# weitianxin/MACR

Measured on AMD Instinct MI355X. Metric: train interactions/sec + eval users/sec (full-catalog top-K@20), higher is better.
Workload: dtype f32; 1 GPU; gowalla-shape MACR-MF rubibceboth d=64 batch=4096 c=40 (n_users=29858, n_items=40981); synthetic Xavier tables, Zipf positives, batches as sampled (grouped on the device inside the step); parallelism=replicas x1 (train) / item-sharded x1 + RCCL all-gather (eval), global_batch=4096

## Files before the change

### macr_amd/csrc/eval_kernels.hip

```cpp
#include "common.hpp"

#include <algorithm>

#include <type_traits>

namespace macr {

#ifdef MACR_ABL_COUNT
__device__ unsigned long long g_dbg[8];
#define MACR_DBG_ADD(k, v) do { if ((threadIdx.x & 63) == 0) atomicAdd(&g_dbg[k], (unsigned long long)(v)); } while (0)
#else
#define MACR_DBG_ADD(k, v) do { } while (0)
#endif

typedef float f32x16 __attribute__((ext_vector_type(16)));

constexpr int kCap = 64;
constexpr int kTileItems = 32;
constexpr int kUnitK = 64;
constexpr int kUnitStride = kUnitK + 1;
constexpr int kWavesPerBlock = 8;
constexpr int kUsersPerBlock = 32 * kWavesPerBlock;
constexpr int kSelRegs = 16;

// ... 1055 lines not shown
        if (has_next) store_tile(buf ^ 1);
        __syncthreads();
#pragma unroll
        for (int g = 0; g < UG; ++g) tm_cur[g] = tm_next[g];
        buf ^= 1;
        t = tn; ++vi;
        if (stop) break;
    }
    for (int k = tid; k < kUsersPerBlock; k += THREADS) {
        const int qq = ub * kUsersPerBlock + k;
        const int ql2 = (REPAIR && rl.compact) ? ubv * kUsersPerBlock + k : qq;
        if (qq < U) counts[(size_t)split * rl.stride + ql2] = (int32_t)min(s_cnt[k], (uint32_t)cap);
    }
    }
}

template <int D>
struct StreamCfgC {
    static constexpr int RU = 2 * D / 8 + 1;
    static constexpr int TU = kTileItems * RU;
    static constexpr int NS = D / 16;
    static constexpr int LDU = (TU + 511) / 512, REM = TU - 512 * (LDU - 1);
    static constexpr size_t smem = (size_t)2 * TU * 16 + kUsersPerBlock * 4 + 16;
};
static inline size_t items_c_bytes(int n_local, int d) { return (size_t)n_tiles(n_local) * kTileItems * (2 * d / 8 + 1) * 16; }
template <int D>
struct StreamCfgH1 {
    static constexpr int RU = D / 8 + 1;
    static constexpr int TU = kTileItems * RU;
    static constexpr int NS = D / 16;
    static constexpr int LDU = (TU + 511) / 512, REM = TU - 512 * (LDU - 1);
    static constexpr size_t smem = (size_t)2 * TU * 16 + kUsersPerBlock * 4 + 16;
};
#ifndef MACR_H_TPS
#define MACR_H_TPS 1
#endif
constexpr int kHTiles = MACR_H_TPS;
template <int D>
struct StreamCfgH {
    static constexpr int RU = D / 8 + 1;
    static constexpr int TU = kTileItems * RU;
    static constexpr int NS = D / 16;
    static constexpr int THREADS = 256 * kHTiles;
    static constexpr int SU = kHTiles * TU;
    static constexpr int LDU = (SU + THREADS - 1) / THREADS;
    static constexpr size_t smem = (size_t)2 * SU * 16 + kUsersPerBlock * 4 + 16;
};
__device__ __forceinline__ f32x16 mfma_f16(bf16x8 a, bf16x8 b, f32x16 acc) {
    return __builtin_amdgcn_mfma_f32_32x32x16_f16(__builtin_bit_cast(f16x8, a), __builtin_bit_cast(f16x8, b), acc, 0, 0, 0);
}

template <int KIND> __device__ __forceinline__ bf16x8 bias_query_unit_h(float su, bool on) {
    const float sv = KIND == MACR_SCORE_DIRECT_MINUS_BOTH ? su : 1.0f;
    const uint32_t s1 = f16_rne_bits(sv);
    const float r1 = sv - f16_bits_value(s1);
    const uint32_t s2 = f16_rne_bits(r1), s3 = f16_rne_bits(r1 - f16_bits_value(s2));
    union { uint32_t u[4]; bf16x8 v; } w;
    w.u[0] = on ? (s1 | (s2 << 16)) : 0u; w.u[1] = on ? (s1 | (s3 << 16)) : 0u; w.u[2] = on ? (s2 | (s1 << 16)) : 0u; w.u[3] = 0u;
    return w.v;
}
__device__ __forceinline__ uint4 bias_item_unit_h(float bias) {
    const float bc = fminf(fmaxf(bias, -kHalfMax), kHalfMax);
    const uint32_t b1 = f16_rne_bits(bc);
    const float r1 = bc - f16_bits_value(b1);
    const uint32_t b2 = f16_rne_bits(r1), b3 = f16_rne_bits(r1 - f16_bits_value(b2));
    return make_uint4(b1 | (b1 << 16), b2 | (b1 << 16), b2 | (b3 << 16), 0u);
}
template <int KIND> __device__ __forceinline__ float query_factor_h(float su) { return KIND == MACR_SCORE_RUBI_BOTH ? su : 1.0f; }

template <int KIND> __device__ __forceinline__ float item_scale_c(float sgi) {
    return (KIND == MACR_SCORE_RUBI_BOTH || KIND == MACR_SCORE_RUBI) ? sgi : 1.0f;
}
template <int KIND> __device__ __forceinline__ float item_bias_c(float sgi, float c) {
    return KIND == MACR_SCORE_NORMAL ? 0.0f : -(c * sgi);
}
__device__ __forceinline__ bool sig_u_tiny(float su) { return !(su > 1e-30f); }

template <int D, int KIND, int TRIPS, bool HALF = false, bool FUSED = false>
// ... 523 lines not shown
            one_visit(std::integral_constant<int, 0>(), t, tm_cur);
            store_tile(std::integral_constant<int, 1>());
            __syncthreads();
            tm_cur = tm_next; t = tn; ++vi;
        }
        if (vi >= i1) break;
        {
            const int tn = vi + 1 < i1 ? visit_after(t) : t;
            load_tile(tn);
            __builtin_amdgcn_sched_barrier(0);
            one_visit(std::integral_constant<int, 1>(), t, tm_cur);
            store_tile(std::integral_constant<int, 0>());
            __syncthreads();
            tm_cur = tm_next; t = tn; ++vi;
        }
    }
    if (q_ok && !merge_pairs) {
        float *o = maxima + ((size_t)split * U + q) * 32;
#pragma unroll
        for (int g = 0; g < 4; ++g)
            *reinterpret_cast<float4 *>(o + 8 * g + 4 * h) = make_float4(cmax[4 * g] * fu, cmax[4 * g + 1] * fu, cmax[4 * g + 2] * fu, cmax[4 * g + 3] * fu);
    }
    if (q_ok && merge_pairs) {
        float *o = maxima + ((size_t)split * U + q) * 16 + 8 * h;
        *reinterpret_cast<float4 *>(o) = make_float4(fmaxf(cmax[0], cmax[8]) * fu, fmaxf(cmax[1], cmax[9]) * fu, fmaxf(cmax[2], cmax[10]) * fu,
                                                     fmaxf(cmax[3], cmax[11]) * fu);
        *reinterpret_cast<float4 *>(o + 4) = make_float4(fmaxf(cmax[4], cmax[12]) * fu, fmaxf(cmax[5], cmax[13]) * fu, fmaxf(cmax[6], cmax[14]) * fu,
                                                         fmaxf(cmax[7], cmax[15]) * fu);
    }
    }
}

template <int D, int KIND, bool REPAIR = false>
__global__ __launch_bounds__(StreamCfgH<D>::THREADS, D <= 64 ? 4 : 2) void k_score_stream_h(
    int U, int n_local, const uint4 *__restrict__ users_h, const uint4 *__restrict__ items_h,
    const float *__restrict__ unorm, const uint32_t *__restrict__ qmax_bits,
    const float *__restrict__ sig_u, float c_val, const float *__restrict__ c_dev,
    const uint32_t *__restrict__ mask_bits, const uint32_t *__restrict__ zero_word, int item_offset, int ublocks,
    const float *__restrict__ tau, uint64_t *__restrict__ lists, int32_t *__restrict__ counts, int cap, int32_t *overflow,
    int ovf_per_user, int32_t *blk_flag, const int32_t *__restrict__ ub_map, const int32_t *__restrict__ n_ub_dev, int slots_full) {
    using C = StreamCfgH<D>;
    constexpr int THREADS = C::THREADS, NS = C::NS, RU = C::RU, TU = C::TU, SU = C::SU, LDU = C::LDU;
    constexpr int kCheckTiles = 8;
    const float c = c_dev ? *c_dev : c_val;
    extern __shared__ __align__(16) unsigned char smem[];
    uint4 *s_t = reinterpret_cast<uint4 *>(smem);
    uint32_t *s_cnt = reinterpret_cast<uint32_t *>(smem + (size_t)2 * SU * 16);
    int *s_stop = reinterpret_cast<int *>(s_cnt + kUsersPerBlock);
    const int tid = threadIdx.x, lane = tid & 63, wid = tid >> 6;
    const int col = lane & 31, h = lane >> 5;
    const int tslot = kHTiles == 2 ? __builtin_amdgcn_readfirstlane(wid >> 2) : 0, uw = wid & 3;
    const int T = (n_local + kTileItems - 1) / kTileItems;
    int n_ub = ublocks;
    long long G = gridDim.x;
    const long long b = blockIdx.x;
    RepairLayout rl = {false, 0, U};
    if (REPAIR) {
        n_ub = *n_ub_dev;
        if (n_ub == 0) return;
        rl = repair_layout(slots_full, U, n_ub);
        G = repair_grid(rl, G, ublocks, n_ub, T);
        if (b >= G) return;
    }
    int S = (int)(0.6180339f * (float)T);
    S = S < 1 ? 1 : S;
    for (;; ++S) {
        int x = S, y = T;
        while (y) { const int r = x % y; x = y; y = r; }
        if (x == 1) break;
    }
    auto visit = [&](int i) { return (int)(((unsigned long long)i * (unsigned)S) % (unsigned)T); };
    auto visit_after = [&](int tile) { const int n = tile + S; return n >= T ? n - T : n; };
    const float qmax = __uint_as_float(*qmax_bits);
    const long long W = (long long)n_ub * T;
    const long long w_end = W * (b + 1) / G;
    const size_t mask_stride = mask_bits ? (size_t)U : 0;
    for (long long w = W * b / G; w < w_end;) {
    const int ubv = (int)(w / T), i0 = (int)(w - (long long)ubv * T);
    const int i1 = (int)min((long long)T, i0 + (w_end - w));
    w += i1 - i0;
    long long first = (long long)ubv * T * G / W;
    while (W * (first + 1) / G <= (long long)ubv * T) ++first;
    while (W * first / G > (long long)ubv * T) --first;
    const int split = (int)(b - first);
    const int ub = REPAIR ? ub_map[ubv] : ubv;
    __syncthreads();
    for (int k = tid; k < kUsersPerBlock; k += THREADS) s_cnt[k] = 0u;
    if (tid == 0) *s_stop = 0;
    bf16x8 bq[2][NS], bext[2];
    float thr[2], fu[2];
    uint32_t my_list[2], my_q[2];
    uint32_t *my_cnt[2];
#pragma unroll
    for (int g = 0; g < 2; ++g) {
        const int uslot = uw * 64 + g * 32 + col, q = ub * kUsersPerBlock + uslot;
        const bool q_ok = q < U;
        const uint4 *urow = users_h + (size_t)(q_ok ? q : 0) * (D / 8);
#pragma unroll
        for (int sI = 0; sI < NS; ++sI) {
            uint4 v = urow[2 * sI + h];
            if (!q_ok) v = make_uint4(0u, 0u, 0u, 0u);
            bq[g][sI] = *reinterpret_cast<bf16x8 *>(&v);
        }
        const float su = (score_uses_sig_u(KIND) && q_ok) ? sig_u[q] : 1.0f;
        const bool tiny = KIND == MACR_SCORE_RUBI_BOTH && sig_u_tiny(su);
        fu[g] = query_factor_h<KIND>(su);
        bext[g] = bias_query_unit_h<KIND>(su, KIND != MACR_SCORE_NORMAL && h == 0);
        float tau_s = __builtin_nanf("");
        if (q_ok) tau_s = tau[q] - 1.01f * filter_margin_h(D, unorm[q], qmax, c) * fu[g];
        thr[g] = tau_s / fu[g];
        if (tiny) thr[g] = q_ok ? -INFINITY : thr[g];
        my_list[g] = (uint32_t)((size_t)split * rl.stride + ((REPAIR && rl.compact) ? ubv * kUsersPerBlock + uslot : (q_ok ? q : 0)));
        my_q[g] = mask_bits ? (uint32_t)(q_ok ? q : 0) : 0u;
        my_cnt[g] = &s_cnt[uslot];
    }
    const int id_lane = item_offset + 4 * h;

    uint4 stg[LDU];
    uint32_t tm_next[2] = {0u, 0u};
    auto load_step = [&](int ta, int tb) {
        const int tau_ = __builtin_amdgcn_readfirstlane(ta), tbu = __builtin_amdgcn_readfirstlane(tb);
#pragma unroll
        for (int k = 0; k < LDU; ++k) {
            int e = tid + THREADS * k;
            if (k + 1 == LDU && e >= SU) e -= SU;
            const bool second = kHTiles == 2 && e >= TU;
            stg[k] = items_h[(size_t)(second ? tbu : tau_) * TU + (second ? e - TU : e)];
        }
        const int mine = tslot ? tbu : tau_;
#ifndef MACR_ABL_H_NOMASK
        const uint32_t *mrow = (mask_bits ? mask_bits : zero_word) + (size_t)mine * mask_stride;
        tm_next[0] = mrow[my_q[0]];
        tm_next[1] = mrow[my_q[1]];
#else
        tm_next[0] = zero_word[mine & 0]; tm_next[1] = tm_next[0];
#endif
    };
    auto store_step = [&](auto BUF) {
        constexpr int buf = decltype(BUF)::value;
#pragma unroll
        for (int k = 0; k < LDU; ++k) {
            asm volatile("" : "+v"(stg[k].x), "+v"(stg[k].y), "+v"(stg[k].z), "+v"(stg[k].w));
            if (k + 1 < LDU || tid < SU - THREADS * (LDU - 1)) s_t[buf * SU + tid + THREADS * k] = stg[k];
        }
    };
    auto one_step = [&](auto BUF, int t, uint32_t tm0, uint32_t tm1) {
        constexpr int buf = decltype(BUF)::value;
        const __bf16 *ua = reinterpret_cast<const __bf16 *>(s_t + buf * SU + tslot * TU) + (size_t)col * (8 * RU) + 8 * h;
        f32x16 acc0, acc1;
#pragma unroll
        for (int r = 0; r < 16; ++r) { acc0[r] = 0.f; acc1[r] = 0.f; }
        constexpr int CH = NS < 2 ? NS : (D <= 64 ? 2 : 4);
        bf16x8 ae;
        if (KIND != MACR_SCORE_NORMAL) ae = *reinterpret_cast<const bf16x8 *>(ua - 8 * h + D);
#pragma unroll
        for (int s0 = 0; s0 < NS; s0 += CH) {
            bf16x8 af[CH];
#pragma unroll
            for (int j = 0; j < CH; ++j) af[j] = *reinterpret_cast<const bf16x8 *>(ua + 16 * (s0 + j));
            asm volatile("s_waitcnt lgkmcnt(0)" ::: "memory");
            __builtin_amdgcn_sched_barrier(0);
#pragma unroll
            for (int j = 0; j < CH; ++j) {
#ifndef MACR_ABL_H_NOMFMA
                acc0 = mfma_f16(af[j], bq[0][s0 + j], acc0);
                acc1 = mfma_f16(af[j], bq[1][s0 + j], acc1);
#else
                acc0[j] += (float)af[j][0] * (float)bq[0][s0 + j][0];
                acc1[j] += (float)af[j][1] * (float)bq[1][s0 + j][1];
#endif
            }
            if (KIND != MACR_SCORE_NORMAL && s0 + CH >= NS) {
                acc0 = mfma_f16(ae, bext[0], acc0);
                acc1 = mfma_f16(ae, bext[1], acc1);
            }
            __builtin_amdgcn_sched_barrier(0);
        }
        const int valid = t < 0 ? 0 : n_local - t * kTileItems;
        const uint32_t tailm = valid < kTileItems ? ~0u << (valid > 0 ? valid : 0) : 0u;
        const int id0 = t * kTileItems + id_lane;
        auto epilogue = [&](const f32x16 &acc, uint32_t tm_cur, float thr_g, float fu_g, uint32_t *cnt_g, uint32_t list_g) {
            const uint32_t tmh = (tm_cur | tailm) >> (4 * h);
#pragma unroll
            for (int r4 = 0; r4 < 16; r4 += 4) {
                const float quad = fmaxf(fmaxf(fmaxf(acc[r4], acc[r4 + 1]), acc[r4 + 2]), acc[r4 + 3]);
                if (!__builtin_amdgcn_ballot_w64(quad >= thr_g)) continue;
#pragma unroll
                for (int r = r4; r < r4 + 4; ++r) {
                    const bool above = acc[r] >= thr_g;
                    if (__builtin_amdgcn_ballot_w64(above)) {
                        const int rbit = (r & 3) + 8 * (r >> 2);
                        uint32_t m = tmh;
                        asm volatile("" : "+v"(m));
                        if (above && !((m >> rbit) & 1u)) {
                            const uint32_t pos = atomicAdd(cnt_g, 1u);
                            if (pos < (uint32_t)cap) lists[(size_t)list_g * cap + pos] = make_key(acc[r] * fu_g, id0 + rbit);
                        }
                    }
                }
            }
        };
#ifndef MACR_ABL_H_NOEPI
        epilogue(acc0, tm0, thr[0], fu[0], my_cnt[0], my_list[0]);
        epilogue(acc1, tm1, thr[1], fu[1], my_cnt[1], my_list[1]);
#else
        {
            float m0 = acc0[0], m1 = acc1[0];
#pragma unroll
            for (int r = 1; r < 16; ++r) { m0 = fmaxf(m0, acc0[r]); m1 = fmaxf(m1, acc1[r]); }
            if (m0 == 1.2345e30f || m1 == 1.2345e30f) epilogue(acc0, tm0, thr[0], fu[0], my_cnt[0], my_list[0]);
        }
#endif
    };
    int polled = 0;
    auto stale_mark = [&](int done_before, int done) -> bool {
        if (!blk_flag) return false;
        auto crossed = [&](int v) { return done_before < v && done >= v; };
        const bool check = crossed(2) || crossed(kCheckTiles) || crossed(4 * kCheckTiles);
        if (!(check || (done >> 3) != (done_before >> 3))) return false;
        bool mine = false;
        if (check) {
            uint32_t a = tslot == 0 ? s_cnt[uw * 64 + lane] : 0u;
#pragma unroll
            for (int m = 32; m >= 1; m >>= 1) a += __shfl_xor(a, m, kWave);
            const float usable = 64.f * (float)(done * kTileItems) * (float)(kSelRegs * 64) / (float)n_local;
            mine = tslot == 0 && (float)a > usable + 128.f;
        } else if (tid == 0) {
            mine = polled != 0;
            polled = __hip_atomic_load(blk_flag + ub, __ATOMIC_RELAXED, __HIP_MEMORY_SCOPE_AGENT);
        }
        if (mine) *s_stop = 1;
        return true;
    };
    auto stale_read = [&](bool looked) -> bool {
        if (!looked) return false;
        const bool stop = *s_stop != 0;
        if (stop && tid == 0) __hip_atomic_store(blk_flag + ub, 1, __ATOMIC_RELAXED, __HIP_MEMORY_SCOPE_AGENT);
        return stop;
    };

    int vi = i0;
    auto second_of = [&](int first_tile, int v) { return (kHTiles == 2 && v + 1 < i1) ? visit_after(first_tile) : -1; };
    auto first_after = [&](int a_, int b_, int v) { return v + kHTiles < i1 ? visit_after(b_ < 0 ? a_ : b_) : a_; };
    int ta = visit(i0), tb = second_of(ta, vi);
    if (vi < i1) { load_step(ta, tb < 0 ? ta : tb); store_step(std::integral_constant<int, 0>()); }
    uint32_t tm0 = tm_next[0], tm1 = tm_next[1];
    __syncthreads();
    while (vi < i1) {
        {
            const int na = first_after(ta, tb, vi), nb = second_of(na, vi + kHTiles);
            load_step(na, nb < 0 ? na : nb);
            __builtin_amdgcn_sched_barrier(0);
            one_step(std::integral_constant<int, 0>(), tslot ? tb : ta, tm0, tm1);
            const int done = min(vi + kHTiles, i1) - i0;
            const bool looked = stale_mark(vi - i0, done);
            store_step(std::integral_constant<int, 1>());
#ifndef MACR_ABL_H_NOBARRIER
            __syncthreads();
#endif
            tm0 = tm_next[0]; tm1 = tm_next[1]; ta = na; tb = nb; vi += kHTiles;
            if (stale_read(looked)) break;
        }
        if (vi >= i1) break;
        {
            const int na = first_after(ta, tb, vi), nb = second_of(na, vi + kHTiles);
            load_step(na, nb < 0 ? na : nb);
            __builtin_amdgcn_sched_barrier(0);
            one_step(std::integral_constant<int, 1>(), tslot ? tb : ta, tm0, tm1);
            const int done = min(vi + kHTiles, i1) - i0;
            const bool looked = stale_mark(vi - i0, done);
            store_step(std::integral_constant<int, 0>());
#ifndef MACR_ABL_H_NOBARRIER
            __syncthreads();
#endif
            tm0 = tm_next[0]; tm1 = tm_next[1]; ta = na; tb = nb; vi += kHTiles;
            if (stale_read(looked)) break;
        }
    }
    for (int k = tid; k < kUsersPerBlock; k += THREADS) {
        const int qq = ub * kUsersPerBlock + k;
        const int ql2 = (REPAIR && rl.compact) ? ubv * kUsersPerBlock + k : qq;
        if (qq < U) {
            counts[(size_t)split * rl.stride + ql2] = (int32_t)min(s_cnt[k], (uint32_t)cap);
            if (s_cnt[k] > (uint32_t)cap) overflow[ovf_per_user ? qq : 0] = 1;
        }
    }
    }
}

template <int D, int KIND, bool HALF = false>
__global__ __launch_bounds__(64) void k_test_bf16_scores(int U, int N, const uint4 *__restrict__ users_c, const uint4 *__restrict__ items_c,
                                                         const float *__restrict__ unorm, const uint32_t *__restrict__ qmax_bits,
                                                         const float *__restrict__ sig_u, float c, float *__restrict__ out,
                                                         float *__restrict__ margin) {
    constexpr int RU = HALF ? D / 8 + 1 : StreamCfgC<D>::RU;
    const int lane = threadIdx.x, col = lane & 31, h = lane >> 5;
    const int item = min((int)blockIdx.x * 32 + col, N - 1), user = min((int)blockIdx.y * 32 + col, U - 1);
    const uint4 *irow = items_c + (size_t)item * RU, *urow = users_c + (size_t)user * (HALF ? D / 8 : 2 * D / 8);
    const float su = score_uses_sig_u(KIND) ? sig_u[user] : 1.0f;
    const bool tiny = score_uses_sig_u(KIND) && sig_u_tiny(su);
    const float fu = HALF ? query_factor_h<KIND>(su) : (KIND == MACR_SCORE_DIRECT_MINUS_BOTH && tiny) ? 1.0f : su;
    const bool ones_on = KIND != MACR_SCORE_NORMAL && h == 0 && !(KIND == MACR_SCORE_DIRECT_MINUS_BOTH && tiny);
    union { uint32_t u[4]; bf16x8 v; } ones;
    ones.u[0] = ones_on ? 0x3f803f80u : 0u; ones.u[1] = ones_on ? 0x00003f80u : 0u; ones.u[2] = 0u; ones.u[3] = 0u;
    if (HALF) ones.v = bias_query_unit_h<KIND>(su, KIND != MACR_SCORE_NORMAL && h == 0);
    f32x16 acc;
#pragma unroll
    for (int r = 0; r < 16; ++r) acc[r] = 0.f;
#pragma unroll
    for (int sI = 0; sI < D / 16; ++sI) {
// ... 1538 lines not shown
}

using namespace macr;

#ifdef MACR_ABL_COUNT
extern "C" void macr_dbg_counters(unsigned long long *out) {
    (void)hipMemcpyFromSymbol(out, HIP_SYMBOL(macr::g_dbg), sizeof(unsigned long long) * 8);
    unsigned long long z[8] = {0};
    (void)hipMemcpyToSymbol(HIP_SYMBOL(macr::g_dbg), z, sizeof(z));
}
#endif

namespace macr {
struct StreamGeo { int ublocks, grid0, slots0, grid1, slots1, range1, grid_h; };
static StreamGeo stream_geo(int U, int n_local, int d) {
    StreamGeo g;
    g.ublocks = (U + kUsersPerBlock - 1) / kUsersPerBlock;
    const int resident = d <= 64 ? 512 : 256;
    const int T1 = (n_local + kTileItems - 1) / kTileItems, sl = sample_log2(n_local), T0 = (T1 + (1 << sl) - 1) >> sl;
    auto plan = [&](int T, int &grid, int &slots) {
        const long long W = (long long)g.ublocks * T;
        long long G = resident;
        if (G > W / 8) G = W / 8;
        if (G > (long long)g.ublocks * 60) G = (long long)g.ublocks * 60;
        if (G < 1) G = 1;
        const long long chunk = W / G;
        grid = (int)G;
        slots = (int)((T + chunk - 1) / chunk + 1);
    };
    plan(T0, g.grid0, g.slots0);
    plan(T1, g.grid1, g.slots1);
    g.range1 = (int)(((long long)g.ublocks * T1 + g.grid1 - 1) / g.grid1);
    g.grid_h = g.grid1;
    if (kHTiles == 1) {
        const long long W = (long long)g.ublocks * T1;
        long long G = 2LL * resident;
        if (G > W / 8) G = W / 8;
        if (G > (long long)g.ublocks * 60) G = (long long)g.ublocks * 60;
        if (G < 1) G = 1;
        const long long chunk = W / G;
        g.grid_h = (int)G;
        g.slots1 = std::max(g.slots1, (int)((T1 + chunk - 1) / chunk + 1));
    }
    return g;
}

struct TopkWs {
    float *tau, *maxima; int32_t *counts; int32_t *overflow, *user_ovf, *ub_map, *blk_flag; uint32_t *shared_thr, *mask_bits; uint64_t *lists;
    uint4 *users_bf, *items_bf; float *unorm;
    uint4 *users_c, *items_c;
    float *qpart;
    int cap; size_t header_bytes, maxima_bytes, mask_bytes, lists_bytes, bytes;
};
static TopkWs carve_topk_ws(void *base, int U, int n_local, const StreamGeo &g, int d = 0) {
    TopkWs w;
    char *p = static_cast<char *>(base);
    size_t off = 0;
    auto take = [&](size_t bytes) { void *r = p ? p + off : nullptr; off += align_up(bytes, 256); return r; };
    w.cap = g.slots1 <= 2 ? 1024 : 512;
    w.counts = static_cast<int32_t *>(take((size_t)g.slots1 * U * 4));
    w.overflow = static_cast<int32_t *>(take(256));
    w.shared_thr = static_cast<uint32_t *>(take((size_t)U * 4));
    w.user_ovf = static_cast<int32_t *>(take((size_t)U * 4));
    w.ub_map = static_cast<int32_t *>(take((size_t)g.ublocks * 4));
    w.blk_flag = static_cast<int32_t *>(take((size_t)g.ublocks * 4));
    w.header_bytes = off;
    w.tau = static_cast<float *>(take((size_t)U * 4));
// ... 266 lines not shown
            MACR_CHECK_LAUNCH("score_sample_b", st);
            launch_k_tau<false>((geo.slots0 * per_c + 63) / 64, sel_blocks, st, U, geo.slots0, K, ws.maxima, nullptr, ws.tau, ws.unorm, qmax_bits, c, c_dev, D,
                                merge_pairs ? 4 : 5, half ? 1 : 0, (half && KIND == MACR_SCORE_RUBI_BOTH) ? sig_u : nullptr);
            MACR_CHECK_LAUNCH("tau", st);
        } else if (seeded && filter_bf16) {
        } else if (seeded) {
            k_tau_seed<D, KIND><<<(U + 7) / 8, 256, 0, st>>>(U, n_local, users_tab, user_ids, items, sig_u, sig_i, c, c_dev,
                                                               mask_bits, item_offset, K, seed_idx, ws.tau, nullptr, 0, nullptr, mask_ptr, mask_idx);
            MACR_CHECK_LAUNCH("tau_seed", st);
        } else if (!list_all && f32_sample_bf16) {
            k_bf16_prep_c<D, KIND, true><<<bf16_prep_c_blocks(U, n_local, D, kPrepTripsAlone), 256, 0, st>>>(U, n_local, users_tab, user_ids, items, sig_u, sig_i, c, c_dev,
                                                                                            ws.users_c, ws.items_c, ws.unorm, qmax_bits);
            MACR_CHECK_LAUNCH("bf16_prep_c", st);
            auto pass0c = k_score_sample_c<D, KIND, false, true>;
            const size_t smem_c = StreamCfgH1<D>::smem;
            MACR_REQUIRE(hipFuncSetAttribute(reinterpret_cast<const void *>(pass0c), hipFuncAttributeMaxDynamicSharedMemorySize,
                                             (int)smem_c) == hipSuccess, MACR_E_LAUNCH, "score_topk: cannot reserve %zu B of LDS", smem_c);
            pass0c<<<geo.grid0, 512, smem_c, st>>>(U, n_local, ws.users_c, ws.items_c, sig_u, mask_bits, zero_word,
                                                  geo.ublocks, ws.maxima, sample_log2(n_local), merge_pairs, nullptr, nullptr, nullptr, 0, nullptr);
            MACR_CHECK_LAUNCH("score_sample_b", st);
            launch_k_tau<false>((geo.slots0 * per_c + 63) / 64, sel_blocks, st, U, geo.slots0, K, ws.maxima, nullptr, ws.tau, ws.unorm, qmax_bits, c, c_dev, D,
                                merge_pairs ? 4 : 5, 1, KIND == MACR_SCORE_RUBI_BOTH ? sig_u : nullptr);
            MACR_CHECK_LAUNCH("tau", st);
        } else if (!list_all) {
            pass0<<<geo.grid0, 512, smem, st>>>(U, n_local, users_tab, user_ids, items, sig_u, sig_i, c, c_dev, mask_bits, item_offset,
                                                geo.ublocks, ws.tau, ws.maxima, ws.lists, ws.counts, ws.cap, ws.overflow, 0,
                                                sample_log2(n_local), nullptr, nullptr, nullptr, SweepArgs{}, 0);
            MACR_CHECK_LAUNCH("score_sample", st);
            launch_tau(false);
            MACR_CHECK_LAUNCH("tau", st);
        }
        if (filter_bf16) {
            const void *pass1c = half ? reinterpret_cast<const void *>(k_score_stream_h<D, KIND>) : reinterpret_cast<const void *>(k_score_stream_c<D, KIND>);
            const size_t smem_c = half ? StreamCfgH<D>::smem : StreamCfgC<D>::smem;
            MACR_REQUIRE(hipFuncSetAttribute(pass1c, hipFuncAttributeMaxDynamicSharedMemorySize,
                                             (int)smem_c) == hipSuccess, MACR_E_LAUNCH, "score_topk: cannot reserve %zu B of LDS", smem_c);
            if (half)
                k_score_stream_h<D, KIND><<<geo.grid_h, StreamCfgH<D>::THREADS, smem_c, st>>>(U, n_local, users_c, ws.items_c, ws.unorm, qmax_bits, sig_u, c, c_dev,
                                                                       mask_bits, zero_word, item_offset, geo.ublocks,
                                                                       ws.tau, ws.lists, ws.counts, ws.cap,
                                                                       repair ? ws.user_ovf : ws.overflow, repair ? 1 : 0,
                                                                       seeded ? ws.blk_flag : nullptr, nullptr, nullptr, 0);
            else
                k_score_stream_c<D, KIND><<<geo.grid1, 512, smem_c, st>>>(U, n_local, users_c, ws.items_c, ws.unorm, qmax_bits, sig_u, c, c_dev,
                                                                       mask_bits, zero_word, item_offset, geo.ublocks,
                                                                       ws.tau, ws.lists, ws.counts, ws.cap,
                                                                       repair ? ws.user_ovf : ws.overflow, repair ? 1 : 0,
                                                                       seeded ? ws.blk_flag : nullptr, nullptr, nullptr, 0);
            MACR_CHECK_LAUNCH("score_stream_b", st);
            k_select_b<D, KIND><<<sel_blocks, 64 * kSelWaves, 0, st>>>(U, n_local, geo.slots1, n_splits, K, ws.cap, ws.lists, ws.counts,
                                                                      repair ? ws.user_ovf : ws.overflow, repair ? 1 : 0, nullptr,
                                                                      seeded ? ws.blk_flag : nullptr, users_tab, user_ids, items,
                                                                      sig_u, sig_i, c, c_dev, item_offset, ws.unorm, qmax_bits,
                                                                      out_val, out_idx, seed_out, half ? 1 : 0);
            MACR_CHECK_LAUNCH("select_b", st);
        } else {
        pass1<<<geo.grid1, 512, smem, st>>>(U, n_local, users_tab, user_ids, items, sig_u, sig_i, c, c_dev, mask_bits, item_offset,
                                            geo.ublocks, ws.tau, ws.maxima, ws.lists, ws.counts, ws.cap,
                                            repair ? ws.user_ovf : ws.overflow, repair ? 1 : 0, 0, nullptr, nullptr,
                                            seeded ? ws.blk_flag : nullptr, SweepArgs{}, 0);
        MACR_CHECK_LAUNCH("score_stream", st);
        k_select<false><<<sel_blocks, 64 * kSelWaves, 0, st>>>(U, geo.slots1, n_splits, K, ws.cap, ws.lists, ws.counts,
                                                              repair ? ws.user_ovf : ws.overflow, repair ? 1 : 0, nullptr,
                                                              seeded ? ws.blk_flag : nullptr, out_val, out_idx, seed_out);
        MACR_CHECK_LAUNCH("select", st);
        }
        if (repair) {
            k_repair_plan<<<geo.ublocks, kUsersPerBlock, 0, st>>>(U, K, geo.slots1, ws.user_ovf, out_val, ws.tau, ws.counts,
                                                                 ws.ub_map, ws.blk_flag, ws.overflow + 1, ws.overflow + 2,
                                                                 first_only ? stats : nullptr);
            MACR_CHECK_LAUNCH("repair_plan", st);
        }
        }
        if (repair) {
            if (first_only) {
            } else if (filter_bf16) {
                auto pass0rb = half ? k_score_sample_c<D, KIND, true, true> : k_score_sample_c<D, KIND, true, false>;
                const void *pass1rc = half ? reinterpret_cast<const void *>(k_score_stream_h<D, KIND, true>) : reinterpret_cast<const void *>(k_score_stream_c<D, KIND, true>);
                const size_t smem_c0 = half ? StreamCfgH1<D>::smem : StreamCfgC<D>::smem, smem_c = half ? StreamCfgH<D>::smem : StreamCfgC<D>::smem;
                hipError_t eb = hipFuncSetAttribute(reinterpret_cast<const void *>(pass0rb), hipFuncAttributeMaxDynamicSharedMemorySize, (int)smem_c0);
                if (eb == hipSuccess) eb = hipFuncSetAttribute(pass1rc, hipFuncAttributeMaxDynamicSharedMemorySize, (int)smem_c);
                MACR_REQUIRE(eb == hipSuccess, MACR_E_LAUNCH, "score_topk: cannot reserve %zu B of LDS", smem_c);
                if (seeded) {
                    pass0rb<<<geo.grid0, 512, smem_c0, st>>>(U, n_local, users_c, ws.items_c, sig_u, mask_bits, zero_word,
                                                            geo.ublocks, ws.maxima, sample_log2(n_local), merge_pairs, ws.ub_map, ws.overflow + 1,
                                                            nullptr, 0, nullptr);
                    MACR_CHECK_LAUNCH("score_sample2", st);
                    launch_k_tau<true>((geo.slots0 * per_c + 63) / 64, sel_blocks, st, U, geo.slots0, K, ws.maxima, ws.blk_flag, ws.tau, ws.unorm, qmax_bits, c, c_dev, D,
                                       merge_pairs ? 4 : 5, half ? 1 : 0, (half && KIND == MACR_SCORE_RUBI_BOTH) ? sig_u : nullptr);
                    MACR_CHECK_LAUNCH("tau2", st);
                }
                if (half)
                    k_score_stream_h<D, KIND, true><<<geo.grid_h, StreamCfgH<D>::THREADS, smem_c, st>>>(U, n_local, users_c, ws.items_c, ws.unorm, qmax_bits, sig_u, c, c_dev,
                                                                                mask_bits, zero_word, item_offset, geo.ublocks, ws.tau,
                                                                                ws.lists, ws.counts, ws.cap, ws.overflow, 0, nullptr,
                                                                                ws.ub_map, ws.overflow + 1, geo.slots1);
                else
                    k_score_stream_c<D, KIND, true><<<geo.grid1, 512, smem_c, st>>>(U, n_local, users_c, ws.items_c, ws.unorm, qmax_bits, sig_u, c, c_dev,
                                                                                mask_bits, zero_word, item_offset, geo.ublocks, ws.tau,
                                                                                ws.lists, ws.counts, ws.cap, ws.overflow, 0, nullptr,
                                                                                ws.ub_map, ws.overflow + 1, geo.slots1);
                MACR_CHECK_LAUNCH("score_stream2", st);
                k_select_b<D, KIND, true><<<sel_blocks, 64 * kSelWaves, 0, st>>>(U, n_local, geo.slots1, n_splits, K, ws.cap, ws.lists,
                                                                                ws.counts, ws.overflow, 0, ws.overflow + 1, ws.blk_flag,
                                                                                users_tab, user_ids, items, sig_u, sig_i, c, c_dev,
                                                                                item_offset, ws.unorm, qmax_bits, out_val, out_idx, seed_out, half ? 1 : 0);
                MACR_CHECK_LAUNCH("select2", st);
            } else {
            if (seeded) {
                pass0r<<<geo.grid0, 512, smem, st>>>(U, n_local, users_tab, user_ids, items, sig_u, sig_i, c, c_dev, mask_bits,
                                                     item_offset, geo.ublocks, ws.tau, ws.maxima, ws.lists, ws.counts, ws.cap,
                                                     ws.overflow, 0, sample_log2(n_local), ws.ub_map, ws.overflow + 1, nullptr, SweepArgs{}, 0);
                MACR_CHECK_LAUNCH("score_sample2", st);
                launch_tau(true);
                MACR_CHECK_LAUNCH("tau2", st);
            }
            pass1r<<<geo.grid1, 512, smem, st>>>(U, n_local, users_tab, user_ids, items, sig_u, sig_i, c, c_dev, mask_bits, item_offset,
                                                 geo.ublocks, ws.tau, ws.maxima, ws.lists, ws.counts, ws.cap, ws.overflow, 0, 0,
                                                 ws.ub_map, ws.overflow + 1, nullptr, SweepArgs{}, geo.slots1);
            MACR_CHECK_LAUNCH("score_stream2", st);
            k_select<true><<<sel_blocks, 64 * kSelWaves, 0, st>>>(U, geo.slots1, n_splits, K, ws.cap, ws.lists, ws.counts, ws.overflow, 0,
                                                           ws.overflow + 1, ws.blk_flag, out_val, out_idx, seed_out);
            MACR_CHECK_LAUNCH("select2", st);
            }
        }
    });
// ... 509 lines not shown
```

Measured before the change: 123.9 million interactions/s.

## Restructure half-precision stream kernel to process two tiles per 256-thread block step

The half-precision scoring stream kernel now keeps 256 threads and has each wave process one or two item tiles per barrier step, instead of spreading two tiles across a 512-thread block. Global loads for the next step are split into phases and interleaved with the MFMA work of the current tiles. Tile and mask pointers advance through incremental cursors. The tail mask is precomputed once, and the stale-check polling is gated by a next-check counter. The aim is to amortise barriers and hide load latency, at the cost of more registers per thread and more complex load scheduling. The direct-minus-both kind at d<=64 keeps one tile.

```diff
diff --git a/macr_amd/csrc/eval_kernels.hip b/macr_amd/csrc/eval_kernels.hip
--- a/macr_amd/csrc/eval_kernels.hip
+++ b/macr_amd/csrc/eval_kernels.hip
@@ -1111,18 +1111,22 @@
     static constexpr int LDU = (TU + 511) / 512, REM = TU - 512 * (LDU - 1);
     static constexpr size_t smem = (size_t)2 * TU * 16 + kUsersPerBlock * 4 + 16;
 };
-#ifndef MACR_H_TPS
-#define MACR_H_TPS 1
+#ifndef MACR_H_WTILES
+#define MACR_H_WTILES 2
 #endif
-constexpr int kHTiles = MACR_H_TPS;
-template <int D>
+constexpr int kHTiles = MACR_H_WTILES;
+static_assert(kHTiles == 1 || kHTiles == 2, "k_score_stream_h stages one or two tiles per step");
+template <int D, int KIND>
+constexpr int h_tiles() { return (D <= 64 && KIND == MACR_SCORE_DIRECT_MINUS_BOTH) ? 1 : kHTiles; }
+template <int D, int HT>
 struct StreamCfgH {
     static constexpr int RU = D / 8 + 1;
     static constexpr int TU = kTileItems * RU;
     static constexpr int NS = D / 16;
-    static constexpr int THREADS = 256 * kHTiles;
-    static constexpr int SU = kHTiles * TU;
+    static constexpr int THREADS = 256;
+    static constexpr int SU = HT * TU;
     static constexpr int LDU = (SU + THREADS - 1) / THREADS;
+    static constexpr int FR = TU / THREADS, R = TU - THREADS * FR;
     static constexpr size_t smem = (size_t)2 * SU * 16 + kUsersPerBlock * 4 + 16;
 };
 __device__ __forceinline__ f32x16 mfma_f16(bf16x8 a, bf16x8 b, f32x16 acc) {
@@ -1712,25 +1716,43 @@
 }
 
 template <int D, int KIND, bool REPAIR = false>
-__global__ __launch_bounds__(StreamCfgH<D>::THREADS, D <= 64 ? 4 : 2) void k_score_stream_h(
+__global__ __launch_bounds__(256, D <= 64 ? 4 : 2) void k_score_stream_h(
     int U, int n_local, const uint4 *__restrict__ users_h, const uint4 *__restrict__ items_h,
     const float *__restrict__ unorm, const uint32_t *__restrict__ qmax_bits,
     const float *__restrict__ sig_u, float c_val, const float *__restrict__ c_dev,
     const uint32_t *__restrict__ mask_bits, const uint32_t *__restrict__ zero_word, int item_offset, int ublocks,
     const float *__restrict__ tau, uint64_t *__restrict__ lists, int32_t *__restrict__ counts, int cap, int32_t *overflow,
     int ovf_per_user, int32_t *blk_flag, const int32_t *__restrict__ ub_map, const int32_t *__restrict__ n_ub_dev, int slots_full) {
-    using C = StreamCfgH<D>;
-    constexpr int THREADS = C::THREADS, NS = C::NS, RU = C::RU, TU = C::TU, SU = C::SU, LDU = C::LDU;
+    constexpr int HT = h_tiles<D, KIND>();
+    using C = StreamCfgH<D, HT>;
+    constexpr int THREADS = C::THREADS, NS = C::NS, RU = C::RU, TU = C::TU, SU = C::SU, LDU = C::LDU, FR = C::FR, R = C::R;
     constexpr int kCheckTiles = 8;
     const float c = c_dev ? *c_dev : c_val;
     extern __shared__ __align__(16) unsigned char smem[];
     uint4 *s_t = reinterpret_cast<uint4 *>(smem);
     uint32_t *s_cnt = reinterpret_cast<uint32_t *>(smem + (size_t)2 * SU * 16);
     int *s_stop = reinterpret_cast<int *>(s_cnt + kUsersPerBlock);
-    const int tid = threadIdx.x, lane = tid & 63, wid = tid >> 6;
+    const int tid = threadIdx.x, lane = tid & 63, uw = tid >> 6;
     const int col = lane & 31, h = lane >> 5;
-    const int tslot = kHTiles == 2 ? __builtin_amdgcn_readfirstlane(wid >> 2) : 0, uw = wid & 3;
     const int T = (n_local + kTileItems - 1) / kTileItems;
+    const float n_local_f = __uint_as_float(__builtin_amdgcn_readfirstlane(__float_as_uint((float)n_local)));
+    const int tail_items = n_local - (T - 1) * kTileItems;
+    const int t_tail = tail_items < kTileItems ? T - 1 : -1;
+    const uint32_t tailm = tail_items < kTileItems ? ~0u << tail_items : 0u;
+    bool ld_b[LDU];
+    uint32_t ld_off[LDU], ld_dst[LDU];
+#pragma unroll
+    for (int k = 0; k < LDU; ++k) {
+        int sec = 0, unit = 0;
+        if (k < FR) { unit = tid + THREADS * k; }
+        else if (k < HT * FR) { sec = 1; unit = tid + THREADS * (k - FR); }
+        else {
+            const int r = tid + THREADS * (k - HT * FR);
+            if (r < R) unit = THREADS * FR + r;
+            else if (r < HT * R) { sec = 1; unit = THREADS * FR + r - R; }
+        }
+        ld_b[k] = sec != 0; ld_off[k] = (uint32_t)unit * 16u; ld_dst[k] = ld_off[k] + (uint32_t)(sec * TU * 16);
+    }
     int n_ub = ublocks;
     long long G = gridDim.x;
     const long long b = blockIdx.x;
@@ -1750,11 +1772,19 @@
         if (x == 1) break;
     }
     auto visit = [&](int i) { return (int)(((unsigned long long)i * (unsigned)S) % (unsigned)T); };
-    auto visit_after = [&](int tile) { const int n = tile + S; return n >= T ? n - T : n; };
     const float qmax = __uint_as_float(*qmax_bits);
     const long long W = (long long)n_ub * T;
     const long long w_end = W * (b + 1) / G;
     const size_t mask_stride = mask_bits ? (size_t)U : 0;
+    const uint32_t *const mask_base = mask_bits ? mask_bits : zero_word;
+    struct Cursor { int t; const uint4 *it; const uint32_t *mr; };
+    const long long it_fwd = (long long)S * TU, it_back = (long long)(S - T) * TU;
+    const long long mr_fwd = (long long)S * (long long)mask_stride, mr_back = (long long)(S - T) * (long long)mask_stride;
+    auto cursor_at = [&](int tile) { return Cursor{tile, items_h + (size_t)tile * TU, mask_base + (size_t)tile * mask_stride}; };
+    auto advanced = [&](const Cursor &cu) {
+        const bool wrap = cu.t + S >= T;
+        return Cursor{cu.t + (wrap ? S - T : S), cu.it + (wrap ? it_back : it_fwd), cu.mr + (wrap ? mr_back : mr_fwd)};
+    };
     for (long long w = W * b / G; w < w_end;) {
     const int ubv = (int)(w / T), i0 = (int)(w - (long long)ubv * T);
     const int i1 = (int)min((long long)T, i0 + (w_end - w));
@@ -1769,8 +1799,8 @@
     if (tid == 0) *s_stop = 0;
     bf16x8 bq[2][NS], bext[2];
     float thr[2], fu[2];
-    uint32_t my_list[2], my_q[2];
-    uint32_t *my_cnt[2];
+    uint32_t my_list, my_q[2];
+    uint32_t *my_cnt = &s_cnt[uw * 64 + col];
 #pragma unroll
     for (int g = 0; g < 2; ++g) {
         const int uslot = uw * 64 + g * 32 + col, q = ub * kUsersPerBlock + uslot;
@@ -1790,49 +1820,66 @@
         if (q_ok) tau_s = tau[q] - 1.01f * filter_margin_h(D, unorm[q], qmax, c) * fu[g];
         thr[g] = tau_s / fu[g];
         if (tiny) thr[g] = q_ok ? -INFINITY : thr[g];
-        my_list[g] = (uint32_t)((size_t)split * rl.stride + ((REPAIR && rl.compact) ? ubv * kUsersPerBlock + uslot : (q_ok ? q : 0)));
-        my_q[g] = mask_bits ? (uint32_t)(q_ok ? q : 0) : 0u;
-        my_cnt[g] = &s_cnt[uslot];
+        if (g == 0) my_list = (uint32_t)((size_t)split * rl.stride + ((REPAIR && rl.compact) ? ubv * kUsersPerBlock + uslot : (q_ok ? q : 0)));
+        my_q[g] = mask_bits ? 4u * (uint32_t)(q_ok ? q : 0) : 0u;
     }
     const int id_lane = item_offset + 4 * h;
 
     uint4 stg[LDU];
-    uint32_t tm_next[2] = {0u, 0u};
-    auto load_step = [&](int ta, int tb) {
-        const int tau_ = __builtin_amdgcn_readfirstlane(ta), tbu = __builtin_amdgcn_readfirstlane(tb);
+    uint32_t tm[2 * HT];
+    Cursor na = cursor_at(0), nb = na;
+    auto phase_of = [](int k) constexpr { return HT == 1 ? 0 : FR == 0 ? (k == 0 ? 0 : 2) : k < FR ? 0 : k < 2 * FR ? 2 : 1; };
+    auto unit_of = [](const uint4 *tile, uint32_t off) {
+        asm volatile("" : "+v"(off));
+        return *reinterpret_cast<const uint4 *>(reinterpret_cast<const char *>(tile) + off);
+    };
+    auto word_of = [](const uint32_t *row, uint32_t off) {
+        asm volatile("" : "+v"(off));
+        return *reinterpret_cast<const uint32_t *>(reinterpret_cast<const char *>(row) + off);
+    };
+    auto plan_step = [&](Cursor &next) { na = next; nb = HT == 2 ? advanced(na) : na; next = advanced(nb); };
+    auto load_rounds = [&](auto PH) {
 #pragma unroll
         for (int k = 0; k < LDU; ++k) {
-            int e = tid + THREADS * k;
-            if (k + 1 == LDU && e >= SU) e -= SU;
-            const bool second = kHTiles == 2 && e >= TU;
-            stg[k] = items_h[(size_t)(second ? tbu : tau_) * TU + (second ? e - TU : e)];
-        }
-        const int mine = tslot ? tbu : tau_;
+            if (decltype(PH)::value >= 0 && phase_of(k) != decltype(PH)::value) continue;
+            if (k < FR || HT == 1 || (k >= 2 * FR && THREADS * (k - 2 * FR + 1) <= R)) stg[k] = unit_of(na.it, ld_off[k]);
+            else if (k < 2 * FR || (THREADS * (k - 2 * FR) >= R && THREADS * (k - 2 * FR + 1) <= 2 * R)) stg[k] = unit_of(nb.it, ld_off[k]);
+            else stg[k] = unit_of(ld_b[k] ? nb.it : na.it, ld_off[k]);
+        }
+    };
+    auto store_rounds = [&](auto BUF, auto PH) {
+        constexpr int buf = decltype(BUF)::value;
+#pragma unroll
+        for (int k = 0; k < LDU; ++k) {
+            if (decltype(PH)::value >= 0 && phase_of(k) != decltype(PH)::value) continue;
+            asm volatile("" : "+v"(stg[k].x), "+v"(stg[k].y), "+v"(stg[k].z), "+v"(stg[k].w));
+            const uint32_t dst = k < FR ? ld_off[k] : k < HT * FR ? ld_off[k] + TU * 16 : ld_dst[k];
+            if (k < HT * FR || tid + THREADS * (k - HT * FR) < HT * R)
+                *reinterpret_cast<uint4 *>(smem + (size_t)buf * SU * 16 + dst) = stg[k];
+        }
+    };
+    auto load_masks = [&](auto SLOT) {
+        constexpr int slot = decltype(SLOT)::value;
 #ifndef MACR_ABL_H_NOMASK
-        const uint32_t *mrow = (mask_bits ? mask_bits : zero_word) + (size_t)mine * mask_stride;
-        tm_next[0] = mrow[my_q[0]];
-        tm_next[1] = mrow[my_q[1]];
+        tm[2 * slot] = word_of(slot ? nb.mr : na.mr, my_q[0]);
+        tm[2 * slot + 1] = word_of(slot ? nb.mr : na.mr, my_q[1]);
 #else
-        tm_next[0] = zero_word[mine & 0]; tm_next[1] = tm_next[0];
+        tm[2 * slot] = zero_word[na.t & 0]; tm[2 * slot + 1] = tm[2 * slot];
 #endif
     };
-    auto store_step = [&](auto BUF) {
-        constexpr int buf = decltype(BUF)::value;
-#pragma unroll
-        for (int k = 0; k < LDU; ++k) {
-            asm volatile("" : "+v"(stg[k].x), "+v"(stg[k].y), "+v"(stg[k].z), "+v"(stg[k].w));
-            if (k + 1 < LDU || tid < SU - THREADS * (LDU - 1)) s_t[buf * SU + tid + THREADS * k] = stg[k];
-        }
-    };
-    auto one_step = [&](auto BUF, int t, uint32_t tm0, uint32_t tm1) {
-        constexpr int buf = decltype(BUF)::value;
-        const __bf16 *ua = reinterpret_cast<const __bf16 *>(s_t + buf * SU + tslot * TU) + (size_t)col * (8 * RU) + 8 * h;
+    auto one_step = [&](auto BUF, auto SLOT, int t, uint32_t tm0, uint32_t tm1, auto mid) {
+        constexpr int buf = decltype(BUF)::value, slot = decltype(SLOT)::value;
+        const __bf16 *ua = reinterpret_cast<const __bf16 *>(s_t + buf * SU + slot * TU) + (size_t)col * (8 * RU) + 8 * h;
+        t = __builtin_amdgcn_readfirstlane(t);
+        const uint32_t past = t == t_tail ? tailm : 0u;
+        tm0 |= past; tm1 |= past;
         f32x16 acc0, acc1;
 #pragma unroll
         for (int r = 0; r < 16; ++r) { acc0[r] = 0.f; acc1[r] = 0.f; }
         constexpr int CH = NS < 2 ? NS : (D <= 64 ? 2 : 4);
+        constexpr bool kLateBias = KIND != MACR_SCORE_NORMAL && D <= 64 && CH == 2;
         bf16x8 ae;
-        if (KIND != MACR_SCORE_NORMAL) ae = *reinterpret_cast<const bf16x8 *>(ua - 8 * h + D);
+        if (KIND != MACR_SCORE_NORMAL && !kLateBias) ae = *reinterpret_cast<const bf16x8 *>(ua - 8 * h + D);
 #pragma unroll
         for (int s0 = 0; s0 < NS; s0 += CH) {
             bf16x8 af[CH];
@@ -1842,6 +1889,11 @@
             __builtin_amdgcn_sched_barrier(0);
 #pragma unroll
             for (int j = 0; j < CH; ++j) {
+                if (kLateBias && s0 + CH >= NS && j == CH - 1) {
+                    __builtin_amdgcn_sched_barrier(0);
+                    ae = *reinterpret_cast<const bf16x8 *>(ua - 8 * h + D);
+                    __builtin_amdgcn_sched_barrier(0);
+                }
 #ifndef MACR_ABL_H_NOMFMA
                 acc0 = mfma_f16(af[j], bq[0][s0 + j], acc0);
                 acc1 = mfma_f16(af[j], bq[1][s0 + j], acc1);
@@ -1851,16 +1903,20 @@
 #endif
             }
             if (KIND != MACR_SCORE_NORMAL && s0 + CH >= NS) {
+                if (kLateBias) {
+                    asm volatile("s_waitcnt lgkmcnt(0)" ::: "memory");
+                    __builtin_amdgcn_sched_barrier(0);
+                }
                 acc0 = mfma_f16(ae, bext[0], acc0);
                 acc1 = mfma_f16(ae, bext[1], acc1);
             }
             __builtin_amdgcn_sched_barrier(0);
         }
-        const int valid = t < 0 ? 0 : n_local - t * kTileItems;
-        const uint32_t tailm = valid < kTileItems ? ~0u << (valid > 0 ? valid : 0) : 0u;
+        mid();
+        __builtin_amdgcn_sched_barrier(0);
         const int id0 = t * kTileItems + id_lane;
-        auto epilogue = [&](const f32x16 &acc, uint32_t tm_cur, float thr_g, float fu_g, uint32_t *cnt_g, uint32_t list_g) {
-            const uint32_t tmh = (tm_cur | tailm) >> (4 * h);
+        auto epilogue = [&](const f32x16 &acc, uint32_t tm_cur, float thr_g, float fu_g, uint32_t *cnt_g, uint32_t list_g, uint32_t list_off) {
+            const uint32_t tmh = tm_cur >> (4 * h);
 #pragma unroll
             for (int r4 = 0; r4 < 16; r4 += 4) {
                 const float quad = fmaxf(fmaxf(fmaxf(acc[r4], acc[r4 + 1]), acc[r4 + 2]), acc[r4 + 3]);
@@ -1874,88 +1930,97 @@
                         asm volatile("" : "+v"(m));
                         if (above && !((m >> rbit) & 1u)) {
                             const uint32_t pos = atomicAdd(cnt_g, 1u);
-                            if (pos < (uint32_t)cap) lists[(size_t)list_g * cap + pos] = make_key(acc[r] * fu_g, id0 + rbit);
+                            if (pos < (uint32_t)cap) lists[(size_t)list_g * cap + (pos + list_off)] = make_key(acc[r] * fu_g, id0 + rbit);
                         }
                     }
                 }
             }
         };
 #ifndef MACR_ABL_H_NOEPI
-        epilogue(acc0, tm0, thr[0], fu[0], my_cnt[0], my_list[0]);
-        epilogue(acc1, tm1, thr[1], fu[1], my_cnt[1], my_list[1]);
+        epilogue(acc0, tm0, thr[0], fu[0], my_cnt, my_list, 0u);
+        epilogue(acc1, tm1, thr[1], fu[1], my_cnt + 32, my_list, 32u * (uint32_t)cap);
 #else
         {
             float m0 = acc0[0], m1 = acc1[0];
 #pragma unroll
             for (int r = 1; r < 16; ++r) { m0 = fmaxf(m0, acc0[r]); m1 = fmaxf(m1, acc1[r]); }
-            if (m0 == 1.2345e30f || m1 == 1.2345e30f) epilogue(acc0, tm0, thr[0], fu[0], my_cnt[0], my_list[0]);
+            if (m0 == 1.2345e30f || m1 == 1.2345e30f) epilogue(acc0, tm0, thr[0], fu[0], my_cnt, my_list, 0u);
         }
 #endif
     };
     int polled = 0;
-    auto stale_mark = [&](int done_before, int done) -> bool {
-        if (!blk_flag) return false;
+    int next_check = blk_flag ? 2 : INT_MAX;
+    auto stale_mark = [&](int done_before, int done) {
         auto crossed = [&](int v) { return done_before < v && done >= v; };
         const bool check = crossed(2) || crossed(kCheckTiles) || crossed(4 * kCheckTiles);
-        if (!(check || (done >> 3) != (done_before >> 3))) return false;
         bool mine = false;
         if (check) {
-            uint32_t a = tslot == 0 ? s_cnt[uw * 64 + lane] : 0u;
+            uint32_t mine_q = tid;
+            asm volatile("" : "+v"(mine_q));
+            uint32_t a = s_cnt[mine_q];
 #pragma unroll
             for (int m = 32; m >= 1; m >>= 1) a += __shfl_xor(a, m, kWave);
-            const float usable = 64.f * (float)(done * kTileItems) * (float)(kSelRegs * 64) / (float)n_local;
-            mine = tslot == 0 && (float)a > usable + 128.f;
+            const float usable = 64.f * (float)(done * kTileItems) * (float)(kSelRegs * 64) / n_local_f;
+            mine = (float)a > usable + 128.f;
         } else if (tid == 0) {
             mine = polled != 0;
             polled = __hip_atomic_load(blk_flag + ub, __ATOMIC_RELAXED, __HIP_MEMORY_SCOPE_AGENT);
         }
         if (mine) *s_stop = 1;
-        return true;
+        next_check = done < kCheckTiles ? kCheckTiles : (done & ~(kCheckTiles - 1)) + kCheckTiles;
     };
-    auto stale_read = [&](bool looked) -> bool {
-        if (!looked) return false;
-        const bool stop = *s_stop != 0;
+    auto stale_read = [&]() -> bool {
+        const bool stop = __builtin_amdgcn_readfirstlane(*s_stop) != 0;
         if (stop && tid == 0) __hip_atomic_store(blk_flag + ub, 1, __ATOMIC_RELAXED, __HIP_MEMORY_SCOPE_AGENT);
         return stop;
     };
 
     int vi = i0;
-    auto second_of = [&](int first_tile, int v) { return (kHTiles == 2 && v + 1 < i1) ? visit_after(first_tile) : -1; };
-    auto first_after = [&](int a_, int b_, int v) { return v + kHTiles < i1 ? visit_after(b_ < 0 ? a_ : b_) : a_; };
-    int ta = visit(i0), tb = second_of(ta, vi);
-    if (vi < i1) { load_step(ta, tb < 0 ? ta : tb); store_step(std::integral_constant<int, 0>()); }
-    uint32_t tm0 = tm_next[0], tm1 = tm_next[1];
+    Cursor next = cursor_at(visit(i0));
+    using I0 = std::integral_constant<int, 0>;
+    using I1 = std::integral_constant<int, 1>;
+    using I2 = std::integral_constant<int, 2>;
+    using All = std::integral_constant<int, -1>;
+    using SlotB = std::integral_constant<int, HT - 1>;
+    plan_step(next);
+    load_rounds(All());
+    load_masks(I0());
+    if (HT == 2) load_masks(SlotB());
+    store_rounds(I0(), All());
+    int ta = na.t, tb = nb.t;
     __syncthreads();
+    auto step = [&](auto BUF) -> bool {
+        constexpr int buf = decltype(BUF)::value;
+        using Other = std::integral_constant<int, 1 - buf>;
+        plan_step(next);
+        load_rounds(I0());
+        __builtin_amdgcn_sched_barrier(0);
+        one_step(BUF, I0(), ta, tm[0], tm[1], [&]() { load_rounds(I1()); });
+        __builtin_amdgcn_sched_barrier(0);
+        load_masks(I0());
+        store_rounds(Other(), I0());
+        store_rounds(Other(), I1());
+        if (HT == 2) {
+            load_rounds(I2());
+            __builtin_amdgcn_sched_barrier(0);
+            if (vi + 1 < i1) one_step(BUF, SlotB(), tb, tm[2 * (HT - 1)], tm[2 * (HT - 1) + 1], []() {});
+            __builtin_amdgcn_sched_barrier(0);
+            load_masks(SlotB());
+        }
+        const int done = min(vi + HT, i1) - i0;
+        const bool looked = done >= next_check;
+        if (looked) stale_mark(vi - i0, done);
+        store_rounds(Other(), I2());
+#ifndef MACR_ABL_H_NOBARRIER
+        __syncthreads();
+#endif
+        ta = na.t; tb = nb.t; vi += HT;
+        return looked && stale_read();
+    };
     while (vi < i1) {
-        {
-            const int na = first_after(ta, tb, vi), nb = second_of(na, vi + kHTiles);
-            load_step(na, nb < 0 ? na : nb);
-            __builtin_amdgcn_sched_barrier(0);
-            one_step(std::integral_constant<int, 0>(), tslot ? tb : ta, tm0, tm1);
-            const int done = min(vi + kHTiles, i1) - i0;
-            const bool looked = stale_mark(vi - i0, done);
-            store_step(std::integral_constant<int, 1>());
-#ifndef MACR_ABL_H_NOBARRIER
-            __syncthreads();
-#endif
-            tm0 = tm_next[0]; tm1 = tm_next[1]; ta = na; tb = nb; vi += kHTiles;
-            if (stale_read(looked)) break;
-        }
+        if (step(std::integral_constant<int, 0>())) break;
         if (vi >= i1) break;
-        {
-            const int na = first_after(ta, tb, vi), nb = second_of(na, vi + kHTiles);
-            load_step(na, nb < 0 ? na : nb);
-            __builtin_amdgcn_sched_barrier(0);
-            one_step(std::integral_constant<int, 1>(), tslot ? tb : ta, tm0, tm1);
-            const int done = min(vi + kHTiles, i1) - i0;
-            const bool looked = stale_mark(vi - i0, done);
-            store_step(std::integral_constant<int, 0>());
-#ifndef MACR_ABL_H_NOBARRIER
-            __syncthreads();
-#endif
-            tm0 = tm_next[0]; tm1 = tm_next[1]; ta = na; tb = nb; vi += kHTiles;
-            if (stale_read(looked)) break;
-        }
+        if (step(std::integral_constant<int, 1>())) break;
     }
     for (int k = tid; k < kUsersPerBlock; k += THREADS) {
         const int qq = ub * kUsersPerBlock + k;
@@ -3560,7 +3625,7 @@
     plan(T1, g.grid1, g.slots1);
     g.range1 = (int)(((long long)g.ublocks * T1 + g.grid1 - 1) / g.grid1);
     g.grid_h = g.grid1;
-    if (kHTiles == 1) {
+    {
         const long long W = (long long)g.ublocks * T1;
         long long G = 2LL * resident;
         if (G > W / 8) G = W / 8;
@@ -3893,11 +3958,11 @@
         }
         if (filter_bf16) {
             const void *pass1c = half ? reinterpret_cast<const void *>(k_score_stream_h<D, KIND>) : reinterpret_cast<const void *>(k_score_stream_c<D, KIND>);
-            const size_t smem_c = half ? StreamCfgH<D>::smem : StreamCfgC<D>::smem;
+            const size_t smem_c = half ? StreamCfgH<D, h_tiles<D, KIND>()>::smem : StreamCfgC<D>::smem;
             MACR_REQUIRE(hipFuncSetAttribute(pass1c, hipFuncAttributeMaxDynamicSharedMemorySize,
                                              (int)smem_c) == hipSuccess, MACR_E_LAUNCH, "score_topk: cannot reserve %zu B of LDS", smem_c);
             if (half)
-                k_score_stream_h<D, KIND><<<geo.grid_h, StreamCfgH<D>::THREADS, smem_c, st>>>(U, n_local, users_c, ws.items_c, ws.unorm, qmax_bits, sig_u, c, c_dev,
+                k_score_stream_h<D, KIND><<<geo.grid_h, StreamCfgH<D, h_tiles<D, KIND>()>::THREADS, smem_c, st>>>(U, n_local, users_c, ws.items_c, ws.unorm, qmax_bits, sig_u, c, c_dev,
                                                                        mask_bits, zero_word, item_offset, geo.ublocks,
                                                                        ws.tau, ws.lists, ws.counts, ws.cap,
                                                                        repair ? ws.user_ovf : ws.overflow, repair ? 1 : 0,
@@ -3938,7 +4003,7 @@
             } else if (filter_bf16) {
                 auto pass0rb = half ? k_score_sample_c<D, KIND, true, true> : k_score_sample_c<D, KIND, true, false>;
                 const void *pass1rc = half ? reinterpret_cast<const void *>(k_score_stream_h<D, KIND, true>) : reinterpret_cast<const void *>(k_score_stream_c<D, KIND, true>);
-                const size_t smem_c0 = half ? StreamCfgH1<D>::smem : StreamCfgC<D>::smem, smem_c = half ? StreamCfgH<D>::smem : StreamCfgC<D>::smem;
+                const size_t smem_c0 = half ? StreamCfgH1<D>::smem : StreamCfgC<D>::smem, smem_c = half ? StreamCfgH<D, h_tiles<D, KIND>()>::smem : StreamCfgC<D>::smem;
                 hipError_t eb = hipFuncSetAttribute(reinterpret_cast<const void *>(pass0rb), hipFuncAttributeMaxDynamicSharedMemorySize, (int)smem_c0);
                 if (eb == hipSuccess) eb = hipFuncSetAttribute(pass1rc, hipFuncAttributeMaxDynamicSharedMemorySize, (int)smem_c);
                 MACR_REQUIRE(eb == hipSuccess, MACR_E_LAUNCH, "score_topk: cannot reserve %zu B of LDS", smem_c);
@@ -3952,7 +4017,7 @@
                     MACR_CHECK_LAUNCH("tau2", st);
                 }
                 if (half)
-                    k_score_stream_h<D, KIND, true><<<geo.grid_h, StreamCfgH<D>::THREADS, smem_c, st>>>(U, n_local, users_c, ws.items_c, ws.unorm, qmax_bits, sig_u, c, c_dev,
+                    k_score_stream_h<D, KIND, true><<<geo.grid_h, StreamCfgH<D, h_tiles<D, KIND>()>::THREADS, smem_c, st>>>(U, n_local, users_c, ws.items_c, ws.unorm, qmax_bits, sig_u, c, c_dev,
                                                                                 mask_bits, zero_word, item_offset, geo.ublocks, ws.tau,
                                                                                 ws.lists, ws.counts, ws.cap, ws.overflow, 0, nullptr,
                                                                                 ws.ub_map, ws.overflow + 1, geo.slots1);
```

Result: no change. 123.2 million interactions/s (-0.5%).
